# FelTris/durf

Measured on AMD Instinct MI355X. Metric: train_rays_per_sec, higher is better.
Workload: dtype bf16

## Files before the change

### durf_amd/_sigs.py

```python
import ctypes as C

vp, i32, f32, u64 = C.c_void_p, C.c_int, C.c_float, C.c_size_t

SIGS = {
    'durf_last_error': (C.c_char_p, []),
    'durf_version': (i32, []),
    'durf_dispatch_seen': (i32, []),
    'durf_dispatch_reset': (i32, []),
    'durf_mlp_param_count': (u64, [i32, i32]),
    'durf_mlp_layer_offset': (u64, [i32, i32, i32, i32]),
    'durf_wpack_fwd_bytes': (u64, [i32]),
    'durf_wpack_bwd_bytes': (u64, [i32]),
    'durf_pack_weights': (i32, [vp, i32, i32, vp, vp, vp]),
    'durf_pack_weights_all': (i32, [vp, vp, i32, vp, vp, i32, vp, u64, i32, vp, vp]),
    'durf_ray_setup': (i32, [vp, i32, i32, vp, vp, vp, vp, vp, vp, vp, vp]),
    'durf_ray_setup_masked': (i32, [vp, i32, i32, vp, vp, vp, vp, vp, vp, vp, vp, vp]),
    'durf_compact_hits': (i32, [vp, i32, i32, vp, vp, vp, vp]),
    'durf_compact_classes': (i32, [vp, i32, i32, i32, vp, vp, vp, vp, vp]),
    'durf_compact_all': (i32, [vp, i32, i32, i32, vp, vp, vp, vp, vp, vp, vp, vp]),
    'durf_ray_prologue': (i32, [vp, i32, i32, i32, vp, vp, vp, vp, vp, vp, vp, vp, vp, vp, vp, vp, vp, i32, vp, vp, vp, u64, C.c_uint32, C.c_uint32, vp]),
    'durf_ray_prologue_pack': (i32, [vp, i32, i32, i32, vp, vp, vp, vp, vp, vp, vp, vp, vp, vp, vp, vp, vp, i32, vp, vp, vp, u64, C.c_uint32, C.c_uint32, vp, vp, i32, vp, vp, i32, vp, u64, i32, vp, vp, vp, u64]),
    'durf_ray_prologue_pack_masked': (i32, [vp, i32, i32, i32, vp, vp, vp, vp, vp, vp, vp, vp, vp, vp, vp, vp, vp, i32, vp, vp, vp, u64, C.c_uint32, C.c_uint32, vp, vp, i32, vp, vp, i32, vp, u64, i32, vp, vp, vp, u64, vp]),
    'durf_sample_t': (i32, [vp, i32, i32, vp, vp, vp, i32, vp]),
    'durf_density_noise': (i32, [vp, u64, vp, f32, vp, C.c_uint32, C.c_uint32, i32]),
# ... 2 lines not shown
    'durf_encode_obj': (i32, [vp, i32, i32, vp, vp, vp, vp, vp, vp, C.POINTER(f32), i32, vp, vp]),
    'durf_mlp_stash_bytes': (u64, [i32, u64]),
    'durf_mlp_mask_bytes': (u64, [u64]),
    'durf_mlp_fwd': (i32, [vp, i32, u64, i32, vp, vp, vp, vp, vp, vp, vp, vp, vp, vp]),
    'durf_mlp_fwd_enc': (i32, [vp, u64, i32, vp, vp, vp, vp, vp, i32, i32, vp, vp, vp, vp, vp, vp, vp, vp, vp, vp, vp]),
    'durf_mlp_fwd_enc_obj': (i32, [vp, u64, i32, vp, vp, vp, vp, vp, i32, i32, vp, vp, vp, vp, vp, vp, vp, vp, vp, vp, vp, i32, vp, vp, C.POINTER(f32), i32, vp, vp, vp, vp, vp, vp]),
    'durf_composite_fwd': (i32, [vp, i32, i32, i32, vp, C.POINTER(vp), vp, vp, vp, f32, i32, vp, vp, vp, vp, vp, vp]),
    'durf_composite_resample': (i32, [vp, i32, i32, i32, vp, C.POINTER(vp), vp, vp, vp, f32, i32, vp, vp, vp, vp, vp, vp, f32, vp, vp, vp, vp, vp, vp, vp, f32, f32, i32, i32, vp, vp, vp, vp]),
    'durf_resample': (i32, [vp, i32, i32, vp, vp, f32, vp, vp]),
    'durf_sorted_piecewise_constant_pdf': (i32, [vp, i32, i32, vp, vp, vp, vp]),
    'durf_loss_prep': (i32, [vp, i32, i32, vp, vp, vp, vp, vp, vp, f32, f32, i32, i32, vp, vp]),
    'durf_loss_bwd': (i32, [vp, i32, i32, i32, vp, C.POINTER(vp), vp, vp, vp, vp, vp, vp, vp, vp, vp, vp, f32, C.POINTER(f32), f32, i32, i32, f32, f32, vp, vp, vp, vp, vp, vp, vp, vp, vp, vp]),
    'durf_loss_bwd_levels': (i32, [vp, i32, i32, i32, i32, vp, vp, vp, vp, vp, vp, vp, vp, vp, f32, f32, i32, f32, f32]),
    'durf_train_stats': (i32, [vp, i32, i32, i32, vp, vp, vp, vp, vp, vp, C.POINTER(vp), C.POINTER(f32), i32, vp, C.POINTER(vp), i32]),
    'durf_mlp_bwd': (i32, [vp, i32, u64, i32, vp, vp, vp, vp, vp, vp, vp, vp, vp, vp, vp]),
    'durf_expand_view': (i32, [vp, u64, i32, vp, vp, vp, vp, vp, vp]),
    'durf_dw_part_floats': (u64, [i32]),
    'durf_dw_bpart_floats': (u64, [i32]),
    'durf_mlp_dw': (i32, [vp, i32, u64, i32, vp, i32, C.POINTER(vp), C.POINTER(vp), C.POINTER(vp), C.POINTER(vp), C.POINTER(vp), vp, vp]),
    'durf_mlp_dw_finalize': (i32, [vp, i32, i32, u64, i32, vp, i32, vp, vp, vp, vp]),
    'durf_mlp_dw_levels': (i32, [vp, i32, i32, C.POINTER(u64), C.POINTER(i32), C.POINTER(vp), C.POINTER(vp), C.POINTER(vp), C.POINTER(vp), C.POINTER(vp), C.POINTER(vp), vp, vp]),
    'durf_mlp_dw_finalize_levels': (i32, [vp, i32, i32, i32, C.POINTER(u64), C.POINTER(i32), C.POINTER(vp), vp, vp, vp, vp]),
    'durf_expand_raw': (i32, [vp, i32, i32, vp, vp, vp, vp, vp]),
    'durf_forward_workspace_bytes': (u64, [i32, i32, i32]),
    'durf_forward': (i32, [vp, vp, vp, u64]),
    'durf_render_image_workspace_bytes': (u64, [i32, i32, i32, i32]),
    'durf_render_image': (i32, [vp, vp, u64, i32, vp, vp, vp, vp, u64]),
    'durf_forward_masked': (i32, [vp, vp, vp, vp, u64]),
    'durf_render_layers_workspace_bytes': (u64, [u64, i32, i32, i32, i32]),
    'durf_render_layers': (i32, [vp, vp, vp, u64, i32, vp, vp, vp, vp, vp, vp, vp, vp, vp, u64]),
# ... 58 lines not shown
```

### durf_amd/csrc/durf_common.h

```cpp
#pragma once
#include <hip/hip_runtime.h>
#include <stdint.h>
#include <algorithm>
#include <cstdlib>
#include <stdio.h>
#include "../../include/durf_hip.h"

typedef __bf16 bf16x8 __attribute__((ext_vector_type(8)));
typedef __bf16 bf16x4 __attribute__((ext_vector_type(4)));
typedef __bf16 bf16x2 __attribute__((ext_vector_type(2)));
typedef float f32x16 __attribute__((ext_vector_type(16)));
typedef float f32x4 __attribute__((ext_vector_type(4)));
typedef float f32x2 __attribute__((ext_vector_type(2)));

#define DURF_WAVE 64

void durf_set_error(const char* fmt, ...);
namespace durf {
void note_dispatch(unsigned bits);
int* next_ticket();
}

#define DURF_CHECK_LAUNCH(name)                                              \
    do {                                                                     \
// ... 143 lines not shown
struct EncIn {
    const float* t_vals; const float* origins_s; const float* dirs_s; const float* radii; const int32_t* hit; int K; int flags;
    int obj; float w[10]; void* view_tile; size_t view_stride;
};
struct BwdStrides { size_t idx, wpack, mask, dz, dz_out, d_enc; };
struct DwStrides { size_t enc, view, stash, dz_out, part, bpart; };

namespace durf {
int launch_pack(void* stream, int width, int in_dim, int K, const float* params, size_t param_stride,
                void* wpack_fwd, void* wpack_bwd);
int launch_encode_obj(void* stream, int K, int max_rays, int N, const int32_t* idx, const int32_t* count,
                      const float* t_vals, const float* origins_s, const float* dirs_s, const float* radii,
                      const float* barf_w, int flags, void* out_tile, size_t out_stride, float* out_f32);
bool obj_msplit(size_t rows);
bool obj_mix(size_t rows);
int launch_mlp_fwd(void* stream, int width, size_t rows, int N, const void* enc_tile, const void* view_bf16,
                   const int32_t* ray_idx, const int32_t* count, const void* wpack_fwd, float* raw, void* stash,
                   void* relu_mask, int K, const FwdStrides& st, const int32_t* tail_idx = nullptr,
                   const int32_t* tail_count = nullptr, const EncIn* enc_in = nullptr);
int launch_mlp_bwd(void* stream, int width, size_t rows, int N, const float* draw, const int32_t* ray_idx,
                   const int32_t* count, const void* wpack_bwd, const void* relu_mask, void* dz, void* dz_out,
                   float* d_enc, int K, const BwdStrides& st, const int32_t* tail_idx = nullptr,
                   const int32_t* tail_count = nullptr, const float* draw_ray_sum = nullptr);
int launch_mlp_bwd_ms_levels(void* stream, size_t rows, int N, int nlevels, const float* const* draw, const int32_t* ray_idx,
                             const int32_t* count, const void* wpack_bwd, const void* const* relu_mask, void* const* dz,
                             void* const* dz_out, int K, const BwdStrides& st);
int launch_expand_view(void* stream, size_t rows, int N, const void* view_bf16, const int32_t* ray_idx,
                       const int32_t* count, void* out_tile, int K, size_t idx_stride, size_t out_stride,
                       const int32_t* tail_idx = nullptr, const int32_t* tail_count = nullptr);
struct DwLevels {
// ... 31 lines not shown
```

### durf_amd/csrc/mlp_bwd.hip

```cpp
#include <stdlib.h>
#include <cstddef>
#include "mlp_pack.h"


template <int W>
__global__ void __launch_bounds__(256)
k_pack_bwd(int in_dim, const float* __restrict__ P, bf16x8* __restrict__ out, size_t p_stride, size_t out_stride) {
    P += blockIdx.y * p_stride;
    out = (bf16x8*)((char*)out + blockIdx.y * out_stride);
    pack_bwd_vec<W>(in_dim, P, out, blockIdx.x * blockDim.x + threadIdx.x);
}

struct BPipe {
    i32x4 rsrc;
    unsigned gnext;
    unsigned lds0;
    char* lds;
    int slot_bytes, par, wave, lane;
    int nw;
    int since;
    __device__ __forceinline__ void skip(int chunks) { gnext += chunks * 1024u; }
    __device__ __forceinline__ void issue(int slot, int chunks) {
        const unsigned dst = lds0 + (unsigned)(slot * slot_bytes);
        for (int c = wave; c < chunks; c += nw)
// ... 379 lines not shown

__global__ void __launch_bounds__(256)
k_mlp_bwd_ms(MsBwd A) {
    extern __shared__ __attribute__((aligned(16))) char smem[];
    const int lane = threadIdx.x & 63;
    const int wave = __builtin_amdgcn_readfirstlane(threadIdx.x >> 6);
    size_t total = 0;
    for (int k = 0; k < A.nobj; k++) total += msb_pairs_of(A, k);
    for (size_t item = blockIdx.x; item < total * (size_t)A.lv.n; item += gridDim.x) {
        int level; size_t k, pair;
        msb_item(A, total, item, level, k, pair);
        msb_bwd_pair(A, A.lv.draw[level], A.lv.relu_mask[level], A.lv.dz[level], A.lv.dz_out[level], smem, lane, wave, true, k, pair);
    }
}

struct BwdKernArgs {
    size_t rows; int N; const float* draw; const int32_t* ray_idx; const int32_t* count; const char* wpack; const uint4* relu_mask;
    bf16x8* dz; bf16x8* dz_out; float* d_enc; BwdStrides bs; const int32_t* tail_idx; const int32_t* tail_count;
    const float* draw_ray_sum; MsBwd ow;
};
__device__ __forceinline__ void mix_object_items_bwd(char* smem, int wave, int nwg) {
    typedef const __attribute__((address_space(4))) char* kptr_t;
    kptr_t ka = (kptr_t)__builtin_amdgcn_kernarg_segment_ptr();
    asm volatile("" : "+s"(ka));
    const unsigned smem_lds = lds_addr_of(smem);
    MsBwd ow;
    load_kernarg(ow, ka + offsetof(BwdKernArgs, ow));
    const int lane = (int)__builtin_amdgcn_mbcnt_hi(~0u, __builtin_amdgcn_mbcnt_lo(~0u, 0u));
    const bool first = wave == MIX_TICKET_WAVE && lane == 0;
    const int half = wave >> 2, w4 = (wave + MIX_ROLE_ROT * half) & 3;
    char* const lds = smem + half * msb::LDS_BYTES;
    volatile __attribute__((address_space(3))) int* const tk =
        (volatile __attribute__((address_space(3))) int*)(size_t)(__builtin_amdgcn_readfirstlane(smem_lds) + 2u * msb::LDS_BYTES);
    volatile __attribute__((address_space(3))) int* const npl = tk + 4;
    if (wave == 0 && lane < ow.nobj) npl[lane] = (int)msb_pairs_of(ow, lane);
// ... 22 lines not shown
        }
        k = (size_t)__builtin_amdgcn_readfirstlane((unsigned)(live ? k : 0));
        const __attribute__((address_space(4))) MsBwd* kp = (const __attribute__((address_space(4))) MsBwd*)(ka + offsetof(BwdKernArgs, ow));
        const float* draw = kp->lv.draw[level];
        const uint4* mk = kp->lv.relu_mask[level];
        bf16x8* dzl = kp->lv.dz[level];
        bf16x8* dzo = kp->lv.dz_out[level];
        msb_bwd_pair(ow, draw, mk, dzl, dzo, lds, lane, w4, live, k, pair);
        if (first) *tk = tn;
        ms_barrier();
        t = __builtin_amdgcn_readfirstlane(*tk);
    }
    if (first && t == last) __hip_atomic_store(ticket, 0, __ATOMIC_RELAXED, __HIP_MEMORY_SCOPE_AGENT);
}

template <int W, bool POSE, int NWV = 8, bool MIX = false>
__global__ void __launch_bounds__(512, 2)
k_mlp_bwd(size_t rows, int N, const float* __restrict__ draw, const int32_t* __restrict__ ray_idx,
          const int32_t* __restrict__ count, const char* __restrict__ wpack,
          const uint4* __restrict__ relu_mask, bf16x8* __restrict__ dz, bf16x8* __restrict__ dz_out,
          float* __restrict__ d_enc, BwdStrides bs, const int32_t* __restrict__ tail_idx,
          const int32_t* __restrict__ tail_count, const float* __restrict__ draw_ray_sum, MsBwd ow_arg) {
    static_assert(!MIX || (W == 256 && NWV == 8 && !POSE), "the mixed launch: background blocks of 8 waves + object items on 2 x 4");
    (void)ow_arg;
    using S = MlpSpec<W>;
    extern __shared__ __attribute__((aligned(16))) char smem[];
    if (gridDim.y > 1) {
        const size_t k = blockIdx.y;
        ray_idx += k * bs.idx;
        count += k;
        wpack += k * bs.wpack;
        relu_mask = (const uint4*)((const char*)relu_mask + k * bs.mask);
        dz = (bf16x8*)((char*)dz + k * bs.dz);
        dz_out = (bf16x8*)((char*)dz_out + k * bs.dz_out);
        if (POSE) d_enc = (float*)((char*)d_enc + k * bs.d_enc);
    }
    size_t nrows = rows;
    if (count) {
        const size_t c = (size_t)(*count) * (size_t)N;
        nrows = c < rows ? c : rows;
    }
    const size_t nrows_c = nrows;
    if (tail_count) {
        const size_t t = nrows_c + (size_t)(*tail_count);
        nrows = t < rows ? t : rows;
    }
    const bool has_block = (size_t)blockIdx.x * (32 * NWV) < nrows;
    if (!MIX && !has_block) return;
    const int lane = threadIdx.x & 63;
    const int wave = __builtin_amdgcn_readfirstlane(threadIdx.x >> 6);
    if (wave >= 4 && has_block) __builtin_amdgcn_s_setprio(1);
    const size_t ntile32 = rows >> 5;
    const size_t nblk = (nrows + 32 * NWV - 1) / (32 * NWV);

    BPipe p;
    constexpr int SLOT = 4 * (S::KW + 1);
    p.rsrc = make_rsrc(wpack);
    p.gnext = 0; p.lds = smem; p.slot_bytes = SLOT * 1024; p.par = 0;
    p.lds0 = (unsigned)(size_t)(__attribute__((address_space(3))) char*)smem;
    p.wave = wave; p.lane = lane; p.nw = NWV;
    constexpr int GB0 = bgroup_tiles(S::CT, 1, SLOT) * 1;
    if (!MIX || has_block) p.issue(0, GB0);

  for (size_t blk = blockIdx.x; blk < nblk; blk += gridDim.x) {
    const bool has_next = blk + gridDim.x < nblk;
    const size_t tile32 = blk * NWV + wave;
    const size_t row = tile32 * 32 + (lane & 31);
    const bool valid = row < nrows;
    const bool tile_valid = tile32 * 32 < nrows;

    f32x4 dr = {0.f, 0.f, 0.f, 0.f};
    if (valid) {
        if (tail_count && row >= nrows_c) {
            dr = *(const f32x4*)(draw_ray_sum + (size_t)tail_idx[row - nrows_c] * 4);
        } else {
            size_t src = row;
            if (ray_idx) src = (size_t)ray_idx[row / (size_t)N] * (size_t)N + row % (size_t)N;
            dr = *(const f32x4*)(draw + src * 4);
        }
    }
    const bf16x8 zero8 = {0, 0, 0, 0, 0, 0, 0, 0};
// ... 634 lines not shown

size_t durf_wpack_bwd_bytes(int width) {
    return (size_t)(width == 256 ? BwdSpec<256>::TOTAL_CHUNKS : BwdSpec<128>::TOTAL_CHUNKS) * 1024;
}

int durf_mlp_bwd(void* stream, int width, size_t rows, int N, const float* draw, const int32_t* ray_idx,
                 const int32_t* count, const void* wpack_bwd, const void* relu_mask, void* dz, void* dz_out,
                 float* d_enc, const int32_t* tail_idx, const int32_t* tail_count, const float* draw_ray_sum) {
    DURF_REQUIRE((tail_idx == nullptr) == (tail_count == nullptr) && (tail_idx == nullptr) == (draw_ray_sum == nullptr),
                 "tail_idx, tail_count and draw_ray_sum go together");
    DURF_REQUIRE(tail_idx == nullptr || (count != nullptr && N % 32 == 0), "tail rows follow a compacted ray list");
    return durf::launch_mlp_bwd(stream, width, rows, N, draw, ray_idx, count, wpack_bwd, relu_mask, dz, dz_out, d_enc,
                                1, BwdStrides{}, tail_idx, tail_count, draw_ray_sum);
}

int durf_obj_bwd_batch_levels(void* stream, int K, int B, int N, int nlevels, const int32_t* idx, const int32_t* count,
                              const float* const* draw, const void* wpack_bwd, const void* const* relu_mask, void* const* dz,
                              void* const* dz_out);
int durf_mlp_bwd_obj(void* stream, size_t rows, int N, const float* draw, const int32_t* ray_idx, const int32_t* count,
                     const void* wpack_bwd, const void* relu_mask, void* dz, void* dz_out, const int32_t* tail_idx,
                     const int32_t* tail_count, const float* draw_ray_sum, int K, int B, int nlevels, const int32_t* obj_idx,
                     const int32_t* obj_count, const float* const* obj_draw, const void* obj_wpack_bwd,
                     const void* const* obj_relu_mask, void* const* obj_dz, void* const* obj_dz_out) {
    DURF_REQUIRE(K > 0 && B > 0 && (size_t)B * N == rows, "K object MLPs over rows = B * N sample rows");
    DURF_REQUIRE(nlevels >= 1 && nlevels <= DURF_MAX_LEVELS, "1 <= nlevels <= DURF_MAX_LEVELS");
    DURF_REQUIRE(obj_idx && obj_count && obj_draw && obj_wpack_bwd && obj_relu_mask && obj_dz && obj_dz_out, "the object launch's buffers");
    const bool mix = durf::obj_mix(rows) && N % 32 == 0 && ray_idx != nullptr && count != nullptr;
    if (!mix) {
        int rc = durf_mlp_bwd(stream, 256, rows, N, draw, ray_idx, count, wpack_bwd, relu_mask, dz, dz_out, nullptr, tail_idx, tail_count,
                              draw_ray_sum);
// ... 345 lines not shown
```

### durf_amd/csrc/mlp_fwd.hip

```cpp
#include <stdlib.h>
#include <cstddef>
#include "mlp_pack.h"
#include "enc_lane.h"


template <int W>
__global__ void __launch_bounds__(256)
k_pack_fwd(int in_dim, const float* __restrict__ P, bf16x8* __restrict__ out, size_t p_stride, size_t out_stride) {
    P += blockIdx.y * p_stride;
    out = (bf16x8*)((char*)out + blockIdx.y * out_stride);
    pack_fwd_vec<W>(in_dim, P, out, blockIdx.x * blockDim.x + threadIdx.x);
}

__global__ void __launch_bounds__(256)
k_pack_all(PackAll a) {
    pack_all_vec(a, (int)blockIdx.y, (int)(blockIdx.x * blockDim.x + threadIdx.x));
}

struct WPipe {
    i32x4 rsrc;
    unsigned gnext;
    unsigned lds0;
    char* lds;
    int slot_bytes;
// ... 969 lines not shown
}

}

namespace durf {

static bool msplit_enabled() {
    const char* e = getenv("DURF_OBJ_MSPLIT");
    return !(e && e[0] == '0');
}
bool obj_msplit(size_t rows) { return rows < (size_t)2048 * 128 && msplit_enabled(); }
bool obj_mix(size_t rows) {
    const char* e = getenv("DURF_OBJ_MIX");
    return !(e && e[0] == '0') && obj_msplit(rows);
}

int pack_bwd_launch(void* stream, int width, int in_dim, int K, const float* params, size_t param_stride, void* wpack_bwd);

int launch_pack(void* stream, int width, int in_dim, int K, const float* params, size_t param_stride,
                void* wpack_fwd, void* wpack_bwd) {
    DURF_REQUIRE(width == 256 || width == 128, "width must be 256 or 128");
    DURF_REQUIRE(in_dim > 0 && in_dim <= DURF_ENC_DIM, "in_dim <= 64");
    if (K <= 0) return 0;
    hipStream_t s = (hipStream_t)stream;
    if (wpack_fwd) {
        const size_t ostride = durf_wpack_fwd_bytes(width);
        if (width == 256)
            hipLaunchKernelGGL(k_pack_fwd<256>, dim3(durf_cdiv(MlpSpec<256>::TOTAL_CHUNKS * 64, 256), K), dim3(256), 0, s,
                               in_dim, params, (bf16x8*)wpack_fwd, param_stride, ostride);
        else
// ... 67 lines not shown
```

### durf_amd/csrc/train.hip

```cpp
#include "durf_common.h"
#include "../../include/durf_hip.h"
#include "side_stream.h"
#include "workspace.h"

namespace {

constexpr int ML = DURF_FORWARD_MAX_LEVELS;
constexpr int OBJ32_NSPLIT = 8;

__global__ void k_tv_rows(int K, const float* __restrict__ pose, const float* __restrict__ prev, float c, float* __restrict__ g) {
    const int i = threadIdx.x, k = i / 3, q = i % 3;
    if (k >= K) return;
    const float t = pose[k * 6 + q] - prev[k * 6 + q];
    const float t2 = c * t;
    g[k * 6 + q] = g[k * 6 + q] + t2;
}

struct TrainWs : durf::RayHeadWs {
    float *norms, *prep, *ray_sums, *sums, *part, *bpart, *opart, *obpart, *scratch, *u_rand, *weight_l2;
    float* draw[ML];
    float *raw_c[ML], *raw_b[ML], *obj_raw[ML], *terms[ML];
    void *wf_bkgd, *wb_bkgd, *wf_obj, *wb_obj, *view_tile, *obj_view_tile;
    void *enc[ML], *stash[ML], *mask[ML], *dz[ML], *dz_out[ML];
    void *obj_enc[ML], *obj_stash[ML], *obj_mask[ML], *obj_dz[ML], *obj_dz_out[ML];
// ... 236 lines not shown
        for (int l = 0; l < L; l++) { dr[l] = w.draw[L - 1 - l]; mk[l] = w.obj_mask[L - 1 - l]; dzl[l] = w.obj_dz[L - 1 - l]; dzo[l] = w.obj_dz_out[L - 1 - l]; }
        STEP(durf_obj_bwd_batch_levels(ov.obj(), K, B, N, L, w.idx_obj, w.count_obj, dr, w.wb_obj, mk, dzl, dzo));
    }
    if (f32o) {
        const float *de[ML], *tv[ML];
        for (int lvl = L - 1; lvl >= 0; lvl--) {
            STEP((x3 ? durf_objf32_bwd_batch_x3 : durf_objf32_bwd_batch)(stream, K, B, N, w.idx_obj, w.count_obj, w.draw[lvl], f.obj_params,
                                                                         f.obj_param_stride, w.obj_ws, w.act32[lvl], w.dz32[lvl],
                                                                         pose_opt ? w.d_enc32[lvl] : nullptr));
            de[L - 1 - lvl] = w.d_enc32[lvl]; tv[L - 1 - lvl] = f.t_vals[lvl];
        }
        if (pose_opt)
            STEP(durf_encode_obj_bwd_levels(stream, K, B, N, L, w.idx_obj, w.count_obj, de, tv, w.o_s, w.d_s, f.radii, f.origins,
                                            f.directions, f.pose, f.barf_w, w.pose_scratch, w.pose_sums, 1, obj_flags));
    }
    for (int lvl = L - 1; lvl >= 0; lvl--) {
        float* rs = K > 0 ? w.ray_sums + (size_t)lvl * B * 4 : nullptr;
        if (mix) {
            const float* dr1[1] = {w.draw[lvl]}; const void* mk1[1] = {w.obj_mask[lvl]};
            void* dz1[1] = {w.obj_dz[lvl]}; void* dzo1[1] = {w.obj_dz_out[lvl]};
            TIMED(DURF_TIMED_BWD + lvl,
                  durf_mlp_bwd_obj(stream, rows, N, w.draw[lvl], w.idx_cls, w.count_cls, w.wb_bkgd, w.mask[lvl], w.dz[lvl], w.dz_out[lvl],
                                   w.idx_cls + B, w.count_cls + 1, rs, K, B, 1, w.idx_obj, w.count_obj, dr1, w.wb_obj, mk1, dz1, dzo1));
        } else if (K > 0) {
            TIMED(DURF_TIMED_BWD + lvl,
                  durf_mlp_bwd(stream, 256, rows, N, w.draw[lvl], w.idx_cls, w.count_cls, w.wb_bkgd, w.mask[lvl], w.dz[lvl], w.dz_out[lvl],
                               nullptr, w.idx_cls + B, w.count_cls + 1, rs));
        } else {
            TIMED(DURF_TIMED_BWD + lvl,
                  durf_mlp_bwd(stream, 256, rows, N, w.draw[lvl], nullptr, nullptr, w.wb_bkgd, w.mask[lvl], w.dz[lvl], w.dz_out[lvl], nullptr,
                               nullptr, nullptr, nullptr));
// ... 133 lines not shown
```

### durf_amd/ops.py

```python
import ctypes as C
import math
import os

import torch

from . import _lib

ENC_DIM = 64
VIEW_DIM = 32


def _stream():
    return torch.cuda.current_stream().cuda_stream


TIMERS = None
TIMED_NAMES = None
TIMERS_ACTIVE = True


class _Timed:
    def __init__(self, name):
        self.name = name

# ... 673 lines not shown

def mlp_bwd(width, rows, N, draw, wpack_bwd, relu_mask, ray_idx=None, count=None, want_d_enc=False,
            tail_idx=None, tail_count=None, draw_ray_sum=None):
    dev = draw.device
    dz = torch.empty(mlp_stash_bytes(width, rows), dtype=torch.uint8, device=dev)
    dz_out = torch.empty(tile_rows(rows), 16, dtype=torch.bfloat16, device=dev)
    d_enc = torch.zeros(rows, ENC_DIM, device=dev) if want_d_enc else None
    with _Timed('mlp_bwd_%d' % width):
        _lib.check(_lib.lib().durf_mlp_bwd(_stream(), width, rows, N, _p(_f32(draw)), _p(ray_idx), _p(count),
                                           _p(wpack_bwd), _p(relu_mask), _p(dz), _p(dz_out), _p(d_enc),
                                           _p(tail_idx), _p(tail_count), _p(draw_ray_sum)),
                   'durf_mlp_bwd')
    return (dz, dz_out, d_enc) if want_d_enc else (dz, dz_out)


def expand_view(rows, N, view_bf16, ray_idx=None, count=None, tail_idx=None, tail_count=None):
    out = torch.empty(tile_rows(rows), VIEW_DIM, dtype=torch.bfloat16, device=view_bf16.device)
    _lib.check(_lib.lib().durf_expand_view(_stream(), rows, N, _p(view_bf16), _p(ray_idx), _p(count),
                                           _p(out), _p(tail_idx), _p(tail_count)), 'durf_expand_view')
    return out


def dw_buffers(width, device):
    part = torch.empty(int(_lib.lib().durf_dw_part_floats(width)), device=device)
    bpart = torch.empty(int(_lib.lib().durf_dw_bpart_floats(width)), device=device)
    return part, bpart


def mlp_dw(width, rows, N, enc_tiles, view_tiles, stashes, dzs, dz_outs, part, bpart, count=None):
    L = len(stashes)
# ... 435 lines not shown
                [('lr', C.c_float), ('max_val', C.c_float), ('max_norm', C.c_float), ('step', C.c_int), ('grad_stats', C.c_void_p),
                 ('flags', C.c_int), ('want_pos', C.c_int), ('want_rot', C.c_int), ('tv_loss_mult', C.c_float),
                 ('comm', C.c_void_p), ('world', C.c_int), ('reduce_stats', C.c_int), ('weight_decay_mult', C.c_float),
                 ('pose_used', C.c_void_p), ('cls_count', C.c_void_p), ('timing', C.c_void_p),
                 ('const_trunk', C.c_void_p), ('const_trunk_valid', C.c_int), ('prefetch_const_trunk', C.c_int)])


TRAIN_OBJ_FP32, TRAIN_POSE_OPT, TRAIN_OBJ_X3 = 1, 2, 4
TIMED_FWD, TIMED_BWD, TIMED_COMPOSITE, TIMED_DW, TIMED_STAGES = 0, 4, 8, 12, 13


class StepTiming(C.Structure):
    _fields_ = [('begin', C.c_void_p * TIMED_STAGES), ('end', C.c_void_p * TIMED_STAGES)]


def _step_timing(num_levels, keep):
    if TIMERS is None or not TIMERS_ACTIVE:
        return None
    want = lambda name: TIMED_NAMES is None or name in TIMED_NAMES
    slots = []
    if want('mlp_fwd_256_train'):
        slots += [('mlp_fwd_256_train', TIMED_FWD + l) for l in range(num_levels)]
    if want('mlp_bwd_256'):
        slots += [('mlp_bwd_256', TIMED_BWD + l) for l in range(num_levels)]
    if want('composite_resample'):
        slots += [('composite_resample', TIMED_COMPOSITE + l) for l in range(num_levels - 1)]
    if want('mlp_dw_256'):
        slots += [('mlp_dw_256', TIMED_DW)]
    if not slots:
        return None
    tm = StepTiming()
    for name, i in slots:
        pair = (_timing_event(), _timing_event())
        tm.begin[i], tm.end[i] = pair[0].cuda_event, pair[1].cuda_event
        TIMERS.setdefault(name, []).append(pair)
    keep.append(tm)
    return tm


# ... 200 lines not shown
    a.adam_m, a.adam_v = _p(_f32(m)), _p(_f32(v))
    a.lr, a.max_val, a.max_norm, a.step = float(lr), float(max_val), float(max_norm), int(step)
    pose_opt = bool(K) and (want_pos or want_rot)
    if pose_opt and not obj_fp32:
        raise NotImplementedError('durf_train_step: DURF_TRAIN_POSE_OPT needs DURF_TRAIN_OBJ_FP32 (csrc/train.hip)')
    a.flags = ((TRAIN_OBJ_FP32 if (K and obj_fp32) else 0) | (TRAIN_POSE_OPT if pose_opt else 0) |
               (TRAIN_OBJ_X3 if (K and obj_fp32 and obj_x3) else 0))
    a.want_pos, a.want_rot, a.tv_loss_mult = int(bool(want_pos)), int(bool(want_rot)), float(tv_loss_mult)
    a.comm, a.world, a.reduce_stats = (comm.handle if comm is not None else None), int(world), int(bool(reduce_stats))
    pose_used = torch.empty_like(pose) if K else None
    cls = torch.empty(8, dtype=torch.int32, device=dev) if K else None
    a.pose_used, a.cls_count = _p(pose_used), _p(cls)
    if const_trunk is not None and K and obj_fp32:
        assert const_trunk.numel() >= 264 and const_trunk.is_contiguous()
        a.const_trunk, a.const_trunk_valid, a.prefetch_const_trunk = _p(_f32(const_trunk)), int(bool(const_trunk_valid)), int(bool(update))
    tm = _step_timing(num_levels, keep) if update else None
    a.timing = C.cast(C.pointer(tm), C.c_void_p) if tm is not None else None
    ws = _workspace(dev, int(L.durf_train_workspace_bytes_flags(B, N, K, num_levels, params_flat.numel(), a.flags)))
    with _Timed('train_call'):
        fn = L.durf_train_step if update else L.durf_loss_backward
        _lib.check(fn(_stream(), C.byref(a), _p(ws), ws.numel()), 'durf_train_step' if update else 'durf_loss_backward')
    return outs, dyn, zo, grad, stats, (gstats if update else None), pose_used, cls
```

### durf_amd/train_boxpose.py

```python
import dataclasses
import math
import struct
from typing import Any

import torch

from . import math as dmath
from . import obbpose_model as om
from . import ops
from . import utils


@dataclasses.dataclass
class TrainState:
    variables: Any
    m: torch.Tensor
    v: torch.Tensor
    step: int = 0


def create_train_state(variables):
    return TrainState(variables, torch.zeros_like(variables.flat), torch.zeros_like(variables.flat), 0)


# ... 234 lines not shown
        res = ops.loss_bwd_levels(lvs, ctx['slot'], ctx['d_s'], pixels, lossmult, gt_depth, sky, dyn, ctx['zo'], float(eps),
                                  float(config.box_loss_mult), bg, model.density_bias, config.disable_multiscale_loss)
        for lvl in range(L):
            draws[lvl], terms[lvl] = res[lvl]
    obj_bwd_done = bool(Kb) and not pose_opt and not f32 and all(d is not None for d in draws)
    obj_bwd_mixed = obj_bwd_done and dd is not None and not obj_side.enabled and ops.obj_mix(rows)
    if obj_bwd_done and not obj_bwd_mixed:
        obj_side.fork()
        with obj_side:
            if obj_side.enabled:
                for d in draws:
                    d.record_stream(obj_side.side)
            order = list(reversed(range(L)))
            ops.obj_bwd_batch_levels([ctx['levels'][l]['slabs'] for l in order], ctx['idx'], ctx['count'],
                                     [draws[l] for l in order], ctx['packs']['obj'][1])
    for lvl in reversed(range(L)):
        lv = ctx['levels'][lvl]
        if prep is None:
            ops.loss_prep(lv['t_vals'], lossmult, gt_depth, sky, dyn, ctx['zo'], float(eps),
                          float(config.box_loss_mult), lvl, config.disable_multiscale_loss, norm=norms[lvl])
        if draws[lvl] is None:
            draw, terms[lvl] = level_loss(lvl)
        else:
            draw = draws[lvl]
        if obj_side.enabled:
            draw.record_stream(obj_side.side)
        if f32:
            fl = lv['f32']
            off = lay.mlp_off['MLP_0']
            dz = ops.mlp_bwd_f32(om.W_BKGD, om.IN_BKGD, rows, N, draw, variables.mlp_flat('MLP_0'), fl['act_b'],
# ... 3 lines not shown
                bkgd_pose_rows(lvl, d_enc, draw)
            ops.mlp_dw_f32(om.W_BKGD, om.IN_BKGD, rows, N, fl['act_b'], dz, grad[off:off + lay.mlp_size[om.W_BKGD]])
        if obj_f32:
            sl = lv['f32']['slabs32']
            o0, sz = lay.mlp_off['BoxMLP_0'], lay.mlp_size[om.W_OBJ]
            ops.objf32_bwd_batch(sl, ctx['idx'], ctx['count'], draw, variables.flat[o0:o0 + K * sz], sz, ctx['obj_ws'],
                                 want_d_enc=pose_opt, x3=ctx.get('obj_x3', False))
            if pose_opt:
                ops.encode_obj_bwd_batch(K, ctx['idx'], ctx['count'], sl.d_enc, lv['t_vals'], ctx['o_s'], ctx['d_s'], radii,
                                         rays.origins, rays.directions, pose_ts, alpha, pose_sums, precise=True,
                                         enc_flags=obj_enc_flags)
        if f32:
            continue
        if not obj_bwd_done:
            obj_side.fork()
        if obj_bwd_mixed:
            dzs[lvl] = ops.mlp_bwd_obj(rows, N, draw, ctx['packs']['MLP_0'][1], lv['mask_b'], dd['idx'][0], dd['count'][0:1],
                                       dd['idx'][1], dd['count'][1:2], ray_sums[lvl], [lv['slabs']], ctx['idx'], ctx['count'],
                                       [draw], ctx['packs']['obj'][1])
        elif dd is not None:
            dzs[lvl] = ops.mlp_bwd(om.W_BKGD, rows, N, draw, ctx['packs']['MLP_0'][1], lv['mask_b'], ray_idx=dd['idx'][0],
                                   count=dd['count'][0:1], tail_idx=dd['idx'][1], tail_count=dd['count'][1:2],
                                   draw_ray_sum=ray_sums[lvl])
        elif hit_rows is not None:
            dz32, d_enc = ops.mlp_bwd_f32(om.W_BKGD, om.IN_BKGD, rows, N, draw, variables.mlp_flat('MLP_0'), lv['f32']['act_hit'],
                                          ray_idx=hit_rows['idx'], count=hit_rows['count'], want_d_enc=True, wstream=ctx['bkgd_ws'])
            hit_dz[lvl] = dz32
            bkgd_pose_rows(lvl, d_enc, draw, denc_slot=hit_rows['slot'])
            draw_rest = torch.where(hit_rows['mask'], 0.0, draw.view(B, N, 4)).reshape(rows, 4)
            dzs[lvl] = ops.mlp_bwd(om.W_BKGD, rows, N, draw_rest, ctx['packs']['MLP_0'][1], lv['mask_b'])
        elif bkgd_pose:
# ... 535 lines not shown
```

### include/durf_ctypes_stub.py

```python
import ctypes as C

vp, i32, f32, u64 = C.c_void_p, C.c_int, C.c_float, C.c_size_t


def bind(path='durf_amd/libdurf_hip.so'):
    L = C.CDLL(path)
    L.durf_last_error.restype = C.c_char_p
    L.durf_last_error.argtypes = []
    L.durf_version.restype = i32
    L.durf_version.argtypes = []
    L.durf_dispatch_seen.restype = i32
    L.durf_dispatch_seen.argtypes = []
    L.durf_dispatch_reset.restype = i32
    L.durf_dispatch_reset.argtypes = []
    L.durf_mlp_param_count.restype = u64
    L.durf_mlp_param_count.argtypes = [i32, i32]
    L.durf_mlp_layer_offset.restype = u64
    L.durf_mlp_layer_offset.argtypes = [i32, i32, i32, i32]
    L.durf_wpack_fwd_bytes.restype = u64
    L.durf_wpack_fwd_bytes.argtypes = [i32]
    L.durf_wpack_bwd_bytes.restype = u64
    L.durf_wpack_bwd_bytes.argtypes = [i32]
    L.durf_pack_weights.restype = i32
    L.durf_pack_weights.argtypes = [vp, i32, i32, vp, vp, vp]
# ... 41 lines not shown
    L.durf_composite_resample.argtypes = [vp, i32, i32, i32, vp, C.POINTER(vp), vp, vp, vp, f32, i32, vp, vp, vp, vp, vp, vp, f32, vp, vp, vp, vp, vp, vp, vp, f32, f32, i32, i32, vp, vp, vp, vp]
    L.durf_resample.restype = i32
    L.durf_resample.argtypes = [vp, i32, i32, vp, vp, f32, vp, vp]
    L.durf_sorted_piecewise_constant_pdf.restype = i32
    L.durf_sorted_piecewise_constant_pdf.argtypes = [vp, i32, i32, vp, vp, vp, vp]
    L.durf_loss_prep.restype = i32
    L.durf_loss_prep.argtypes = [vp, i32, i32, vp, vp, vp, vp, vp, vp, f32, f32, i32, i32, vp, vp]
    L.durf_loss_bwd.restype = i32
    L.durf_loss_bwd.argtypes = [vp, i32, i32, i32, vp, C.POINTER(vp), vp, vp, vp, vp, vp, vp, vp, vp, vp, vp, f32, C.POINTER(f32), f32, i32, i32, f32, f32, vp, vp, vp, vp, vp, vp, vp, vp, vp, vp]
    L.durf_loss_bwd_levels.restype = i32
    L.durf_loss_bwd_levels.argtypes = [vp, i32, i32, i32, i32, vp, vp, vp, vp, vp, vp, vp, vp, vp, f32, f32, i32, f32, f32]
    L.durf_train_stats.restype = i32
    L.durf_train_stats.argtypes = [vp, i32, i32, i32, vp, vp, vp, vp, vp, vp, C.POINTER(vp), C.POINTER(f32), i32, vp, C.POINTER(vp), i32]
    L.durf_mlp_bwd.restype = i32
    L.durf_mlp_bwd.argtypes = [vp, i32, u64, i32, vp, vp, vp, vp, vp, vp, vp, vp, vp, vp, vp]
    L.durf_expand_view.restype = i32
    L.durf_expand_view.argtypes = [vp, u64, i32, vp, vp, vp, vp, vp, vp]
    L.durf_dw_part_floats.restype = u64
    L.durf_dw_part_floats.argtypes = [i32]
    L.durf_dw_bpart_floats.restype = u64
    L.durf_dw_bpart_floats.argtypes = [i32]
    L.durf_mlp_dw.restype = i32
    L.durf_mlp_dw.argtypes = [vp, i32, u64, i32, vp, i32, C.POINTER(vp), C.POINTER(vp), C.POINTER(vp), C.POINTER(vp), C.POINTER(vp), vp, vp]
    L.durf_mlp_dw_finalize.restype = i32
    L.durf_mlp_dw_finalize.argtypes = [vp, i32, i32, u64, i32, vp, i32, vp, vp, vp, vp]
    L.durf_mlp_dw_levels.restype = i32
    L.durf_mlp_dw_levels.argtypes = [vp, i32, i32, C.POINTER(u64), C.POINTER(i32), C.POINTER(vp), C.POINTER(vp), C.POINTER(vp), C.POINTER(vp), C.POINTER(vp), C.POINTER(vp), vp, vp]
    L.durf_mlp_dw_finalize_levels.restype = i32
    L.durf_mlp_dw_finalize_levels.argtypes = [vp, i32, i32, i32, C.POINTER(u64), C.POINTER(i32), C.POINTER(vp), vp, vp, vp, vp]
    L.durf_expand_raw.restype = i32
# ... 129 lines not shown
```

### include/durf_hip.h

```cpp
#ifndef DURF_HIP_H
#define DURF_HIP_H
#include <stddef.h>
#include <stdint.h>

#ifdef __cplusplus
extern "C" {
#endif

#define DURF_MAX_OBJ 16
#define DURF_MAX_LEVELS 8
#define DURF_MAX_CAMS 8
#define DURF_W_BKGD 256
#define DURF_W_OBJ 128
#define DURF_ENC_CONTRACT 1
#define DURF_ENC_NO_INTEGRATION 2
#define DURF_ENC_CYLINDER 4
#define DURF_FWD_RAW_FULL 8
#define DURF_ENC_DIM 64
#define DURF_VIEW_DIM 32

const char* durf_last_error(void);
int durf_version(void);
#define DURF_DISPATCH_FWD256_8W 0x1
#define DURF_DISPATCH_FWD256_4W 0x2
// ... 166 lines not shown
int durf_loss_bwd_levels(void* stream, int B, int N, int K, int L, const durf_loss_level* levels ,
                         const int32_t* slot, const float* dirs_s, const float* pixels, const float* lossmult,
                         const float* gt_depth, const float* sky, const int32_t* dyn, const float* zo, float eps,
                         float box_loss_mult, int disable_multiscale, float bg, float density_bias);

int durf_train_stats(void* stream, int L, int K, int N, const float* norms, float* sums,
                     const float* weight_l2, const float* pose6, const float* prev6, const float* target6,
                     const float* const* t_vals, const float* mults, int mode, float* out,
                     const float* const* terms ,
                     int B);

int durf_mlp_bwd(void* stream, int width, size_t rows, int N, const float* draw, const int32_t* ray_idx,
                 const int32_t* count, const void* wpack_bwd, const void* relu_mask, void* dz, void* dz_out,
                 float* d_enc ,
                 const int32_t* tail_idx, const int32_t* tail_count, const float* draw_ray_sum );
int durf_expand_view(void* stream, size_t rows, int N, const void* view_bf16, const int32_t* ray_idx,
                     const int32_t* count, void* out_tile ,
                     const int32_t* tail_idx, const int32_t* tail_count );

size_t durf_dw_part_floats(int width);
size_t durf_dw_bpart_floats(int width);
int durf_mlp_dw(void* stream, int width, size_t rows, int N, const int32_t* count, int nlevels,
                const void* const* enc_tile, const void* const* view_tile, const void* const* stash,
                const void* const* dz, const void* const* dz_out, float* part, float* bpart);
int durf_mlp_dw_finalize(void* stream, int width, int in_dim, size_t rows, int N, const int32_t* count,
                         int nlevels ,
                         const float* part, const float* bpart, float* grad_mlp,
                         const float* mlp_params );
int durf_mlp_dw_levels(void* stream, int width, int nlevels, const size_t* rows, const int* rows_per_ray,
                       const int32_t* const* count, const void* const* enc_tile, const void* const* view_tile,
// ... 231 lines not shown
```

Before: 991,800.

## Merge per-level background MLP backward launches into one multi-level kernel launch

```diff
diff --git a/durf_amd/_sigs.py b/durf_amd/_sigs.py
--- a/durf_amd/_sigs.py
+++ b/durf_amd/_sigs.py
@@ -40,6 +40,7 @@
     'durf_loss_bwd_levels': (i32, [vp, i32, i32, i32, i32, vp, vp, vp, vp, vp, vp, vp, vp, vp, f32, f32, i32, f32, f32]),
     'durf_train_stats': (i32, [vp, i32, i32, i32, vp, vp, vp, vp, vp, vp, C.POINTER(vp), C.POINTER(f32), i32, vp, C.POINTER(vp), i32]),
     'durf_mlp_bwd': (i32, [vp, i32, u64, i32, vp, vp, vp, vp, vp, vp, vp, vp, vp, vp, vp]),
+    'durf_mlp_bwd_levels': (i32, [vp, u64, i32, i32, C.POINTER(vp), vp, vp, vp, C.POINTER(vp), C.POINTER(vp), C.POINTER(vp), vp, vp, C.POINTER(vp), C.POINTER(vp)]),
     'durf_expand_view': (i32, [vp, u64, i32, vp, vp, vp, vp, vp, vp]),
     'durf_dw_part_floats': (u64, [i32]),
     'durf_dw_bpart_floats': (u64, [i32]),
diff --git a/durf_amd/csrc/durf_common.h b/durf_amd/csrc/durf_common.h
--- a/durf_amd/csrc/durf_common.h
+++ b/durf_amd/csrc/durf_common.h
@@ -181,6 +181,7 @@
                       const float* barf_w, int flags, void* out_tile, size_t out_stride, float* out_f32);
 bool obj_msplit(size_t rows);
 bool obj_mix(size_t rows);
+bool bwd_levels(int width, size_t rows, int nlevels, const float* d_enc);
 int launch_mlp_fwd(void* stream, int width, size_t rows, int N, const void* enc_tile, const void* view_bf16,
                    const int32_t* ray_idx, const int32_t* count, const void* wpack_fwd, float* raw, void* stash,
                    void* relu_mask, int K, const FwdStrides& st, const int32_t* tail_idx = nullptr,
diff --git a/durf_amd/csrc/mlp_bwd.hip b/durf_amd/csrc/mlp_bwd.hip
--- a/durf_amd/csrc/mlp_bwd.hip
+++ b/durf_amd/csrc/mlp_bwd.hip
@@ -417,11 +417,23 @@
     }
 }
 
-struct BwdKernArgs {
+struct BwdLevels {
+    const float* draw[DURF_MAX_LEVELS];
+    const uint4* relu_mask[DURF_MAX_LEVELS];
+    bf16x8* dz[DURF_MAX_LEVELS];
+    bf16x8* dz_out[DURF_MAX_LEVELS];
+    const float* draw_ray_sum[DURF_MAX_LEVELS];
+    int n;
+};
+
+template <class Last>
+struct BwdKernArgsT {
     size_t rows; int N; const float* draw; const int32_t* ray_idx; const int32_t* count; const char* wpack; const uint4* relu_mask;
     bf16x8* dz; bf16x8* dz_out; float* d_enc; BwdStrides bs; const int32_t* tail_idx; const int32_t* tail_count;
-    const float* draw_ray_sum; MsBwd ow;
+    const float* draw_ray_sum; Last ow;
 };
+typedef BwdKernArgsT<MsBwd> BwdKernArgs;
+typedef BwdKernArgsT<BwdLevels> BwdLvKernArgs;
 __device__ __forceinline__ void mix_object_items_bwd(char* smem, int wave, int nwg) {
     typedef const __attribute__((address_space(4))) char* kptr_t;
     kptr_t ka = (kptr_t)__builtin_amdgcn_kernarg_segment_ptr();
@@ -474,18 +486,20 @@
     if (first && t == last) __hip_atomic_store(ticket, 0, __ATOMIC_RELAXED, __HIP_MEMORY_SCOPE_AGENT);
 }
 
-template <int W, bool POSE, int NWV = 8, bool MIX = false>
+template <int W, bool POSE, int NWV = 8, bool MIX = false, bool LV = false>
 __global__ void __launch_bounds__(512, 2)
 k_mlp_bwd(size_t rows, int N, const float* __restrict__ draw, const int32_t* __restrict__ ray_idx,
           const int32_t* __restrict__ count, const char* __restrict__ wpack,
           const uint4* __restrict__ relu_mask, bf16x8* __restrict__ dz, bf16x8* __restrict__ dz_out,
           float* __restrict__ d_enc, BwdStrides bs, const int32_t* __restrict__ tail_idx,
-          const int32_t* __restrict__ tail_count, const float* __restrict__ draw_ray_sum, MsBwd ow_arg) {
+          const int32_t* __restrict__ tail_count, const float* __restrict__ draw_ray_sum,
+          std::conditional_t<LV, BwdLevels, MsBwd> ow_arg) {
     static_assert(!MIX || (W == 256 && NWV == 8 && !POSE), "the mixed launch: background blocks of 8 waves + object items on 2 x 4");
+    static_assert(!LV || (W == 256 && NWV == 8 && !POSE && !MIX), "the levels launch: background blocks of 8 waves only");
     (void)ow_arg;
     using S = MlpSpec<W>;
     extern __shared__ __attribute__((aligned(16))) char smem[];
-    if (gridDim.y > 1) {
+    if (!LV && gridDim.y > 1) {
         const size_t k = blockIdx.y;
         ray_idx += k * bs.idx;
         count += k;
@@ -505,7 +519,13 @@
         const size_t t = nrows_c + (size_t)(*tail_count);
         nrows = t < rows ? t : rows;
     }
-    const bool has_block = (size_t)blockIdx.x * (32 * NWV) < nrows;
+    const __attribute__((address_space(4))) BwdLevels* const lvk = !LV ? nullptr :
+        (const __attribute__((address_space(4))) BwdLevels*)((const __attribute__((address_space(4))) char*)
+                                                              __builtin_amdgcn_kernarg_segment_ptr() + offsetof(BwdLvKernArgs, ow));
+    using blk_t = std::conditional_t<LV, unsigned, size_t>;
+    blk_t nvirt = 0;
+    if constexpr (LV) nvirt = (unsigned)lvk->n * (unsigned)((nrows + 32 * NWV - 1) / (32 * NWV));
+    const bool has_block = LV ? blockIdx.x < nvirt : (size_t)blockIdx.x * (32 * NWV) < nrows;
     if (!MIX && !has_block) return;
     const int lane = threadIdx.x & 63;
     const int wave = __builtin_amdgcn_readfirstlane(threadIdx.x >> 6);
@@ -522,9 +542,18 @@
     constexpr int GB0 = bgroup_tiles(S::CT, 1, SLOT) * 1;
     if (!MIX || has_block) p.issue(0, GB0);
 
-  for (size_t blk = blockIdx.x; blk < nblk; blk += gridDim.x) {
-    const bool has_next = blk + gridDim.x < nblk;
-    const size_t tile32 = blk * NWV + wave;
+  if constexpr (!LV) nvirt = nblk;
+  for (blk_t vblk = blockIdx.x; vblk < nvirt; vblk += gridDim.x) {
+    const bool has_next = vblk + gridDim.x < nvirt;
+    blk_t blk = vblk;
+    if constexpr (LV) {
+        int li = 0;
+        while (blk >= (unsigned)nblk) { blk -= (unsigned)nblk; li++; }
+        li = __builtin_amdgcn_readfirstlane(li);
+        draw = lvk->draw[li]; relu_mask = lvk->relu_mask[li]; dz = lvk->dz[li]; dz_out = lvk->dz_out[li];
+        draw_ray_sum = lvk->draw_ray_sum[li];
+    }
+    const size_t tile32 = (size_t)blk * NWV + wave;
     const size_t row = tile32 * 32 + (lane & 31);
     const bool valid = row < nrows;
     const bool tile_valid = tile32 * 32 < nrows;
@@ -1189,6 +1218,38 @@
                                 1, BwdStrides{}, tail_idx, tail_count, draw_ray_sum);
 }
 
+int durf_mlp_bwd_levels(void* stream, size_t rows, int N, int nlevels, const float* const* draw, const int32_t* ray_idx,
+                        const int32_t* count, const void* wpack_bwd, const void* const* relu_mask, void* const* dz,
+                        void* const* dz_out, const int32_t* tail_idx, const int32_t* tail_count, const float* const* draw_ray_sum,
+                        float* const* d_enc) {
+    DURF_REQUIRE(nlevels >= 1 && nlevels <= DURF_MAX_LEVELS, "1 <= nlevels <= DURF_MAX_LEVELS");
+    DURF_REQUIRE(d_enc == nullptr, "no d(enc) epilogue: the box-pose backward keeps its launch per level (durf_mlp_bwd)");
+    DURF_REQUIRE(draw && relu_mask && dz && dz_out, "the levels' buffers");
+    DURF_REQUIRE((tail_idx == nullptr) == (tail_count == nullptr) && (tail_idx == nullptr) == (draw_ray_sum == nullptr),
+                 "tail_idx, tail_count and draw_ray_sum go together");
+    DURF_REQUIRE(tail_idx == nullptr || (count != nullptr && N % 32 == 0), "tail rows follow a compacted ray list");
+    DURF_REQUIRE(rows % 32 == 0, "rows must be a multiple of 32");
+    DURF_REQUIRE(N >= 1, "N >= 1");
+    BwdLevels lv{};
+    lv.n = nlevels;
+    for (int l = 0; l < nlevels; l++) {
+        DURF_REQUIRE(draw[l] && relu_mask[l] && dz[l] && dz_out[l] && (!draw_ray_sum || draw_ray_sum[l]), "a buffer per level");
+        lv.draw[l] = draw[l]; lv.relu_mask[l] = (const uint4*)relu_mask[l]; lv.dz[l] = (bf16x8*)dz[l]; lv.dz_out[l] = (bf16x8*)dz_out[l];
+        lv.draw_ray_sum[l] = draw_ray_sum ? draw_ray_sum[l] : nullptr;
+    }
+    if (rows == 0) return 0;
+    const size_t nvirt = (size_t)nlevels * durf_cdiv(rows, 256);
+    DURF_REQUIRE(nvirt + 256 < ((size_t)1 << 32), "the levels' 256-sample blocks are counted in 32 bits");
+    constexpr int lds = 2 * 4 * (MlpSpec<256>::KW + 1) * 1024;
+    (void)hipFuncSetAttribute((const void*)k_mlp_bwd<256, false, 8, false, true>, hipFuncAttributeMaxDynamicSharedMemorySize, lds);
+    hipLaunchKernelGGL((k_mlp_bwd<256, false, 8, false, true>), dim3((unsigned)(nvirt < 256 ? nvirt : 256)), dim3(512), lds,
+                       (hipStream_t)stream, rows, N, (const float*)nullptr, ray_idx, count, (const char*)wpack_bwd, (const uint4*)nullptr,
+                       (bf16x8*)nullptr, (bf16x8*)nullptr, (float*)nullptr, BwdStrides{}, tail_idx, tail_count, (const float*)nullptr, lv);
+    DURF_CHECK_LAUNCH("durf_mlp_bwd_levels");
+    durf::note_dispatch(DURF_DISPATCH_BWD256_8W);
+    return 0;
+}
+
 int durf_obj_bwd_batch_levels(void* stream, int K, int B, int N, int nlevels, const int32_t* idx, const int32_t* count,
                               const float* const* draw, const void* wpack_bwd, const void* const* relu_mask, void* const* dz,
                               void* const* dz_out);
diff --git a/durf_amd/csrc/mlp_fwd.hip b/durf_amd/csrc/mlp_fwd.hip
--- a/durf_amd/csrc/mlp_fwd.hip
+++ b/durf_amd/csrc/mlp_fwd.hip
@@ -1007,6 +1007,10 @@
     const char* e = getenv("DURF_OBJ_MIX");
     return !(e && e[0] == '0') && obj_msplit(rows);
 }
+bool bwd_levels(int width, size_t rows, int nlevels, const float* d_enc) {
+    const char* e = getenv("DURF_BWD_LEVELS");
+    return !(e && e[0] == '0') && width == 256 && d_enc == nullptr && nlevels >= 2 && rows >= (size_t)2048 * 128;
+}
 
 int pack_bwd_launch(void* stream, int width, int in_dim, int K, const float* params, size_t param_stride, void* wpack_bwd);
 
diff --git a/durf_amd/csrc/train.hip b/durf_amd/csrc/train.hip
--- a/durf_amd/csrc/train.hip
+++ b/durf_amd/csrc/train.hip
@@ -274,7 +274,19 @@
             STEP(durf_encode_obj_bwd_levels(stream, K, B, N, L, w.idx_obj, w.count_obj, de, tv, w.o_s, w.d_s, f.radii, f.origins,
                                             f.directions, f.pose, f.barf_w, w.pose_scratch, w.pose_sums, 1, obj_flags));
     }
-    for (int lvl = L - 1; lvl >= 0; lvl--) {
+    const bool bwd_lv = !mix && !f32o && durf::bwd_levels(256, rows, L, nullptr);
+    if (bwd_lv) {
+        const float *dr[ML], *rsl[ML]; const void* mk[ML]; void* dzl[ML]; void* dzo[ML];
+        for (int l = 0; l < L; l++) {
+            const int lvl = L - 1 - l;
+            dr[l] = w.draw[lvl]; mk[l] = w.mask[lvl]; dzl[l] = w.dz[lvl]; dzo[l] = w.dz_out[lvl];
+            rsl[l] = w.ray_sums + (size_t)lvl * B * 4;
+        }
+        TIMED(DURF_TIMED_BWD + L - 1,
+              durf_mlp_bwd_levels(stream, rows, N, L, dr, K > 0 ? w.idx_cls : nullptr, K > 0 ? w.count_cls : nullptr, w.wb_bkgd, mk, dzl,
+                                  dzo, K > 0 ? w.idx_cls + B : nullptr, K > 0 ? w.count_cls + 1 : nullptr, K > 0 ? rsl : nullptr, nullptr));
+    }
+    for (int lvl = L - 1; lvl >= 0 && !bwd_lv; lvl--) {
         float* rs = K > 0 ? w.ray_sums + (size_t)lvl * B * 4 : nullptr;
         if (mix) {
             const float* dr1[1] = {w.draw[lvl]}; const void* mk1[1] = {w.obj_mask[lvl]};
diff --git a/durf_amd/ops.py b/durf_amd/ops.py
--- a/durf_amd/ops.py
+++ b/durf_amd/ops.py
@@ -711,6 +711,24 @@
     return (dz, dz_out, d_enc) if want_d_enc else (dz, dz_out)
 
 
+def bwd_levels(rows, num_levels):
+    return os.environ.get('DURF_BWD_LEVELS', '1')[:1] != '0' and num_levels >= 2 and rows >= OVERLAP_MIN_ROWS
+
+
+def mlp_bwd_levels(rows, N, draws, wpack_bwd, relu_masks, ray_idx=None, count=None, tail_idx=None, tail_count=None,
+                   draw_ray_sums=None, d_encs=None):
+    dev = draws[0].device
+    nl = len(draws)
+    dzs = [torch.empty(mlp_stash_bytes(256, rows), dtype=torch.uint8, device=dev) for _ in range(nl)]
+    dz_outs = [torch.empty(tile_rows(rows), 16, dtype=torch.bfloat16, device=dev) for _ in range(nl)]
+    arr = lambda ts: None if ts is None else (C.c_void_p * max(len(ts), 1))(*[t.data_ptr() for t in ts])
+    with _Timed('mlp_bwd_256'):
+        _lib.check(_lib.lib().durf_mlp_bwd_levels(_stream(), rows, N, nl, arr([_f32(d) for d in draws]), _p(ray_idx), _p(count),
+                                                  _p(wpack_bwd), arr(relu_masks), arr(dzs), arr(dz_outs), _p(tail_idx),
+                                                  _p(tail_count), arr(draw_ray_sums), arr(d_encs)), 'durf_mlp_bwd_levels')
+    return list(zip(dzs, dz_outs))
+
+
 def expand_view(rows, N, view_bf16, ray_idx=None, count=None, tail_idx=None, tail_count=None):
     out = torch.empty(tile_rows(rows), VIEW_DIM, dtype=torch.bfloat16, device=view_bf16.device)
     _lib.check(_lib.lib().durf_expand_view(_stream(), rows, N, _p(view_bf16), _p(ray_idx), _p(count),
@@ -1176,7 +1194,7 @@
     _fields_ = [('begin', C.c_void_p * TIMED_STAGES), ('end', C.c_void_p * TIMED_STAGES)]
 
 
-def _step_timing(num_levels, keep):
+def _step_timing(num_levels, keep, bwd_merged=False):
     if TIMERS is None or not TIMERS_ACTIVE:
         return None
     want = lambda name: TIMED_NAMES is None or name in TIMED_NAMES
@@ -1184,7 +1202,7 @@
     if want('mlp_fwd_256_train'):
         slots += [('mlp_fwd_256_train', TIMED_FWD + l) for l in range(num_levels)]
     if want('mlp_bwd_256'):
-        slots += [('mlp_bwd_256', TIMED_BWD + l) for l in range(num_levels)]
+        slots += [('mlp_bwd_256', TIMED_BWD + l) for l in (range(num_levels - 1, num_levels) if bwd_merged else range(num_levels))]
     if want('composite_resample'):
         slots += [('composite_resample', TIMED_COMPOSITE + l) for l in range(num_levels - 1)]
     if want('mlp_dw_256'):
@@ -1415,7 +1433,7 @@
     if const_trunk is not None and K and obj_fp32:
         assert const_trunk.numel() >= 264 and const_trunk.is_contiguous()
         a.const_trunk, a.const_trunk_valid, a.prefetch_const_trunk = _p(_f32(const_trunk)), int(bool(const_trunk_valid)), int(bool(update))
-    tm = _step_timing(num_levels, keep) if update else None
+    tm = _step_timing(num_levels, keep, bwd_merged=not (K and obj_fp32) and bwd_levels(B * N, num_levels)) if update else None
     a.timing = C.cast(C.pointer(tm), C.c_void_p) if tm is not None else None
     ws = _workspace(dev, int(L.durf_train_workspace_bytes_flags(B, N, K, num_levels, params_flat.numel(), a.flags)))
     with _Timed('train_call'):
diff --git a/durf_amd/train_boxpose.py b/durf_amd/train_boxpose.py
--- a/durf_amd/train_boxpose.py
+++ b/durf_amd/train_boxpose.py
@@ -272,6 +272,8 @@
             order = list(reversed(range(L)))
             ops.obj_bwd_batch_levels([ctx['levels'][l]['slabs'] for l in order], ctx['idx'], ctx['count'],
                                      [draws[l] for l in order], ctx['packs']['obj'][1])
+    bwd_merged = (not f32 and not obj_f32 and not bkgd_pose and hit_rows is None and not obj_bwd_mixed and
+                  (obj_bwd_done or not Kb) and all(d is not None for d in draws) and ops.bwd_levels(rows, L))
     for lvl in reversed(range(L)):
         lv = ctx['levels'][lvl]
         if prep is None:
@@ -305,7 +307,16 @@
             continue
         if not obj_bwd_done:
             obj_side.fork()
-        if obj_bwd_mixed:
+        if bwd_merged:
+            if lvl == L - 1:
+                order = list(reversed(range(L)))
+                tails = {} if dd is None else dict(ray_idx=dd['idx'][0], count=dd['count'][0:1], tail_idx=dd['idx'][1],
+                                                   tail_count=dd['count'][1:2], draw_ray_sums=[ray_sums[l] for l in order])
+                res = ops.mlp_bwd_levels(rows, N, [draws[l] for l in order], ctx['packs']['MLP_0'][1],
+                                         [ctx['levels'][l]['mask_b'] for l in order], **tails)
+                for l, r in zip(order, res):
+                    dzs[l] = r
+        elif obj_bwd_mixed:
             dzs[lvl] = ops.mlp_bwd_obj(rows, N, draw, ctx['packs']['MLP_0'][1], lv['mask_b'], dd['idx'][0], dd['count'][0:1],
                                        dd['idx'][1], dd['count'][1:2], ray_sums[lvl], [lv['slabs']], ctx['idx'], ctx['count'],
                                        [draw], ctx['packs']['obj'][1])
diff --git a/include/durf_ctypes_stub.py b/include/durf_ctypes_stub.py
--- a/include/durf_ctypes_stub.py
+++ b/include/durf_ctypes_stub.py
@@ -79,6 +79,8 @@
     L.durf_train_stats.argtypes = [vp, i32, i32, i32, vp, vp, vp, vp, vp, vp, C.POINTER(vp), C.POINTER(f32), i32, vp, C.POINTER(vp), i32]
     L.durf_mlp_bwd.restype = i32
     L.durf_mlp_bwd.argtypes = [vp, i32, u64, i32, vp, vp, vp, vp, vp, vp, vp, vp, vp, vp, vp]
+    L.durf_mlp_bwd_levels.restype = i32
+    L.durf_mlp_bwd_levels.argtypes = [vp, u64, i32, i32, C.POINTER(vp), vp, vp, vp, C.POINTER(vp), C.POINTER(vp), C.POINTER(vp), vp, vp, C.POINTER(vp), C.POINTER(vp)]
     L.durf_expand_view.restype = i32
     L.durf_expand_view.argtypes = [vp, u64, i32, vp, vp, vp, vp, vp, vp]
     L.durf_dw_part_floats.restype = u64
diff --git a/include/durf_hip.h b/include/durf_hip.h
--- a/include/durf_hip.h
+++ b/include/durf_hip.h
@@ -204,6 +204,10 @@
                  const int32_t* count, const void* wpack_bwd, const void* relu_mask, void* dz, void* dz_out,
                  float* d_enc ,
                  const int32_t* tail_idx, const int32_t* tail_count, const float* draw_ray_sum );
+int durf_mlp_bwd_levels(void* stream, size_t rows, int N, int nlevels, const float* const* draw, const int32_t* ray_idx,
+                        const int32_t* count, const void* wpack_bwd, const void* const* relu_mask, void* const* dz,
+                        void* const* dz_out, const int32_t* tail_idx, const int32_t* tail_count,
+                        const float* const* draw_ray_sum, float* const* d_enc);
 int durf_expand_view(void* stream, size_t rows, int N, const void* view_bf16, const int32_t* ray_idx,
                      const int32_t* count, void* out_tile ,
                      const int32_t* tail_idx, const int32_t* tail_count );
```

Result: slower. 975,600 (-1.6%).
